# parsakhaz/multimodal-image-similarity-search

Hardware: AMD Instinct MI355X
Metric: images/s CLIP-B/32 encode @ bs256; Mvec/s cosine top-10 over 10M x 512 (higher is better)
Workload: dtype bf16

## Files before the change

### include/mmiss_debug.h

```cpp
#ifndef MMISS_DEBUG_H
#define MMISS_DEBUG_H
#include <stdint.h>
#ifdef __cplusplus
extern "C" {
#endif

enum {
    MMISS_EPI_F32 = 0,
    MMISS_EPI_BIAS_BF16 = 1,
    MMISS_EPI_BIAS_QGELU_BF16 = 2,
    MMISS_EPI_BIAS_RESID_F32 = 3,
    MMISS_EPI_PATCH_F32 = 4
};

int mmiss_dbg_gemm(int device, void* hip_stream, int epi, int variant, const void* A, const void* W,
                   void* out, const float* bias, const float* aux, int32_t M, int32_t N, int32_t K,
                   int32_t p0, int32_t p1);

int mmiss_dbg_layernorm(int device, void* hip_stream, const float* x, const float* gamma, const float* beta,
                        void* out, int32_t out_bf16, int32_t M, int32_t d, float eps);

int mmiss_dbg_attention(int device, void* hip_stream, const void* qkv, void* ctx, int32_t B, int32_t T,
                        int32_t H, int32_t causal);

int mmiss_dbg_attention_pooled(int device, void* hip_stream, const void* qkv, const int32_t* pool_row, void* ctxc, int32_t B,
                               int32_t T, int32_t H, int32_t causal);

int mmiss_dbg_gemm_resid_rows(int device, void* hip_stream, const void* A, const void* W, float* out, const float* bias,
                              const void* rows_bf16, const int32_t* rowmap, int32_t M, int32_t N, int32_t K);

int mmiss_dbg_patch_from_pixels(int device, void* hip_stream, const float* pixels, const void* W, float* out, const float* pos,
                                int32_t B, int32_t S, int32_t P, int32_t d);

int mmiss_dbg_im2col(int device, void* hip_stream, const float* pixels, void* out, int32_t B, int32_t S,
                     int32_t P, int32_t Kp);

int mmiss_dbg_gemm_time(int device, int epi, int variant, const void* A, const void* W, void* out,
                        const float* bias, const float* aux, int32_t M, int32_t N, int32_t K,
                        int32_t p0, int32_t p1, int32_t iters, float* ms_per_launch);

int mmiss_dbg_gemm_p256(int device, void* hip_stream, int epi, const void* A, const void* W, void* out,
                        const float* bias, const float* aux, const float* ln_stats, float ln_eps, int32_t M, int32_t N,
                        int32_t K, int32_t m_valid, int32_t iters, float* ms_per_launch);

int mmiss_dbg_gemm_resid16(int device, void* hip_stream, int variant, const void* A, const void* W, void* out,
                           const float* bias, float* stats_out, int32_t M, int32_t N, int32_t K, int32_t m_valid,
                           int32_t iters, float* ms_per_launch);

struct mmiss_encoder;
int mmiss_dbg_encoder_record_taps(struct mmiss_encoder* enc, int on);
int mmiss_dbg_encoder_set_fuse_ln(struct mmiss_encoder* enc, int on);

int mmiss_dbg_gemm_split_time(int device, int epi, int bm, const void* A, const void* W, void* out, const float* bias,
                              int32_t M, int32_t N, int32_t K, int32_t iters, float* ms);

int mmiss_dbg_quantize_weights_fp8(int device, void* hip_stream, const void* w_bf16, void* w8, float* scale, int32_t N,
                                   int32_t K);
int mmiss_dbg_layernorm_mxfp8(int device, void* hip_stream, const float* x, const float* gamma, const float* beta,
                              void* out8, void* out_scale, int32_t M, int32_t d, float eps);
int mmiss_dbg_layernorm16_mxfp8(int device, void* hip_stream, const void* x_bf16, const float* gamma, const float* beta,
                                void* out8, void* out_scale, int32_t M, int32_t d, float eps);
int mmiss_dbg_attention_mx(int device, void* hip_stream, const void* qkv, void* ctx8, void* ctx_scale, int32_t B, int32_t T,
                           int32_t H);
int mmiss_dbg_gemm8(int device, void* hip_stream, int epi, int bm, const void* A8, const void* As, const void* W8,
                    const float* wscale, const float* bias, void* out, void* out_scale, int32_t M, int32_t N, int32_t K);
int mmiss_dbg_gemm8_xt(int device, void* hip_stream, int epi, int xt, const void* A8, const void* As, const void* W8,
                       const float* wscale, const float* bias, void* out, void* out_scale, int32_t M, int32_t N, int32_t K,
                       int32_t m_valid, const void* c16, const float* ln_stats, const void* x16, float ln_eps, void* q_out,
                       void* q_scale, float* stats_out);
int mmiss_dbg_quant16_mxfp8_stats(int device, void* hip_stream, const void* x_bf16, void* out8, void* out_scale, float* stats,
                                  int32_t M, int32_t d);
int mmiss_dbg_quantize_weights_fp8_csum(int device, void* hip_stream, const void* w_bf16, void* w8, float* scale, void* c16,
                                        int32_t N, int32_t K);
int mmiss_dbg_gemm8_time(int device, int epi, int bm, const void* A8, const void* As, const void* W8, const float* wscale,
                         const float* bias, void* out, void* out_scale, int32_t M, int32_t N, int32_t K, int32_t iters,
                         float* ms_per_launch);

int mmiss_dbg_set_option(const char* key, int value);

#ifdef __cplusplus
}
#endif
#endif
```

### multimodal-image-similarity-search_amd/_lib.py

```python
from __future__ import annotations

import ctypes as C
import os
import threading

_HERE = os.path.dirname(os.path.abspath(__file__))
LIB_PATH = os.path.join(_HERE, "libmmiss.so")

MMISS_OK = 0
MMISS_F32 = 0
MMISS_F16 = 1
MMISS_F8 = 2
MMISS_PREC_BF16 = 0
MMISS_PREC_FP8 = 1
MMISS_PREC_BF16_F32RESID = 2
MMISS_TOWER_VISION = 0
MMISS_TOWER_TEXT = 1

EPI_F32, EPI_BIAS_BF16, EPI_BIAS_QGELU_BF16, EPI_BIAS_RESID_F32, EPI_PATCH_F32 = range(5)


class MmissError(RuntimeError):

    def __init__(self, code: int, msg: str):
# ... 27 lines not shown
    "mmiss_encoder_set_weight": (_I, [_P, C.c_char_p, _P, _I64, C.POINTER(_I)]),
    "mmiss_encoder_finalize": (_I, [_P]),
    "mmiss_encoder_set_precision": (_I, [_P, _I32]),
    "mmiss_encoder_set_tower_precision": (_I, [_P, _I32, _I32]),
    "mmiss_encoder_set_stream": (_I, [_P, _P, _I32]),
    "mmiss_encode_image": (_I, [_P, _P, _I32, _P]),
    "mmiss_encode_image_u8": (_I, [_P, _P, _I32, _P]),
    "mmiss_resize_crop_rgb": (_I, [_P, _P, _I64, _P, _P, _P, _I32, _P]),
    "mmiss_encode_image_rgb": (_I, [_P, _P, _I64, _P, _P, _P, _I32, _P]),
    "mmiss_encode_text": (_I, [_P, _P, _I32, _I32, _P]),
    "mmiss_encoder_tap": (_I, [_P, _I, _I, _P, _I64, C.POINTER(_I64)]),
    "mmiss_index_create": (_I, [_I32, _I32, _I, _I64, C.POINTER(_P)]),
    "mmiss_index_destroy": (_I, [_P]),
    "mmiss_index_set_stream": (_I, [_P, _P, _I32]),
    "mmiss_index_add": (_I, [_P, _P, _P, _I64]),
    "mmiss_index_update": (_I, [_P, _P, _P, _I64]),
    "mmiss_index_remove": (_I, [_P, _P, _I64, C.POINTER(_I64)]),
    "mmiss_index_clear": (_I, [_P]),
    "mmiss_index_count": (_I, [_P, C.POINTER(_I64)]),
    "mmiss_index_get": (_I, [_P, _P, _I64, _P]),
    "mmiss_index_labels": (_I, [_P, _P, _I64]),
    "mmiss_index_query": (_I, [_P, _P, _I32, _I32, _P, _P, _P]),
    "mmiss_index_query_begin": (_I, [_P, _P, _I32, _I32, _P, _P, _P]),
    "mmiss_index_query_end": (_I, [_P]),
    "mmiss_index_query_abort": (_I, [_P]),
    "mmiss_index_guard_stats": (_I, [_P, C.POINTER(_I64)]),
    "mmiss_index_guard_stats_ex": (_I, [_P, C.POINTER(_I64)]),
    "mmiss_index_save": (_I, [_P, C.c_char_p]),
    "mmiss_index_load": (_I, [_P, C.c_char_p]),
    "mmiss_index_set_tags": (_I, [_P, _P, _P, _I64]),
    "mmiss_index_get_tags": (_I, [_P, _P, _I64, _P]),
    "mmiss_index_query_filtered": (_I, [_P, _P, _I32, _I32, _P, _P, _P, _P, _P]),
    "mmiss_index_query_filtered_begin": (_I, [_P, _P, _I32, _I32, _P, _P, _P, _P, _P]),
    "mmiss_blend": (_I, [_I, _P, _P, _P, C.c_double, _I32, _I32, _P]),
    "mmiss_merge_topk": (_I, [_I, _P, _P, _P, _I32, _I32, _I32, _P, _P, _P]),
    "mmiss_prof_enable": (_I, [_I]),
    "mmiss_prof_filter": (_I, [C.c_char_p, _I]),
    "mmiss_prof_reset": (_I, []),
    "mmiss_prof_read": (_I, [C.c_char_p, C.c_size_t]),
    "mmiss_dbg_gemm": (_I, [_I, _P, _I, _I, _P, _P, _P, _P, _P, _I32, _I32, _I32, _I32, _I32]),
    "mmiss_dbg_gemm_p256": (_I, [_I, _P, _I, _P, _P, _P, _P, _P, _P, C.c_float, _I32, _I32, _I32, _I32, _I32, _P]),
    "mmiss_dbg_gemm_resid16": (_I, [_I, _P, _I, _P, _P, _P, _P, _P, _I32, _I32, _I32, _I32, _I32, _P]),
    "mmiss_dbg_gemm_time": (_I, [_I, _I, _I, _P, _P, _P, _P, _P, _I32, _I32, _I32, _I32, _I32, _I32,
                                 C.POINTER(C.c_float)]),
    "mmiss_dbg_layernorm": (_I, [_I, _P, _P, _P, _P, _P, _I32, _I32, _I32, C.c_float]),
    "mmiss_dbg_attention": (_I, [_I, _P, _P, _P, _I32, _I32, _I32, _I32]),
    "mmiss_dbg_im2col": (_I, [_I, _P, _P, _P, _I32, _I32, _I32, _I32]),
    "mmiss_dbg_patch_from_pixels": (_I, [_I, _P, _P, _P, _P, _P, _I32, _I32, _I32, _I32]),
    "mmiss_dbg_attention_pooled": (_I, [_I, _P, _P, _P, _P, _I32, _I32, _I32, _I32]),
    "mmiss_dbg_gemm_resid_rows": (_I, [_I, _P, _P, _P, _P, _P, _P, _P, _I32, _I32, _I32]),
    "mmiss_dbg_encoder_record_taps": (_I, [_P, _I]),
    "mmiss_dbg_encoder_set_fuse_ln": (_I, [_P, _I]),
    "mmiss_dbg_set_option": (_I, [C.c_char_p, _I]),
    "mmiss_dbg_quantize_weights_fp8": (_I, [_I, _P, _P, _P, _P, _I32, _I32]),
    "mmiss_dbg_layernorm_mxfp8": (_I, [_I, _P, _P, _P, _P, _P, _P, _I32, _I32, C.c_float]),
    "mmiss_dbg_layernorm16_mxfp8": (_I, [_I, _P, _P, _P, _P, _P, _P, _I32, _I32, C.c_float]),
    "mmiss_dbg_attention_mx": (_I, [_I, _P, _P, _P, _P, _I32, _I32, _I32]),
    "mmiss_dbg_gemm8": (_I, [_I, _P, _I, _I, _P, _P, _P, _P, _P, _P, _P, _I32, _I32, _I32]),
    "mmiss_dbg_gemm8_xt": (_I, [_I, _P, _I, _I, _P, _P, _P, _P, _P, _P, _P, _I32, _I32, _I32, _I32, _P, _P, _P, C.c_float, _P, _P, _P]),
    "mmiss_dbg_quant16_mxfp8_stats": (_I, [_I, _P, _P, _P, _P, _P, _I32, _I32]),
    "mmiss_dbg_quantize_weights_fp8_csum": (_I, [_I, _P, _P, _P, _P, _P, _I32, _I32]),
    "mmiss_dbg_gemm8_time": (_I, [_I, _I, _I, _P, _P, _P, _P, _P, _P, _P, _I32, _I32, _I32, _I32, C.POINTER(C.c_float)]),
    "mmiss_dbg_gemm_split_time": (_I, [_I, _I, _I, _P, _P, _P, _P, _I32, _I32, _I32, _I32, C.POINTER(C.c_float)]),
}

_lib = None
_lock = threading.Lock()


def load() -> C.CDLL:
    global _lib
    with _lock:
        if _lib is not None:
            return _lib
        if not os.path.exists(LIB_PATH):
            raise ImportError(
                f"{LIB_PATH} not found: the HIP extension is not built. "
                "Run `python -c 'import __graft_entry__ as g; g.build()'` at the repo root. "
                "There is no CPU fallback for the mmiss hot path."
            )
        lib = C.CDLL(LIB_PATH, mode=C.RTLD_GLOBAL)
        for name, (res, args) in SIGNATURES.items():
            fn = getattr(lib, name)
            fn.restype = res
            fn.argtypes = args
        if lib.mmiss_abi_version() != 1:
            raise ImportError("libmmiss.so ABI version mismatch")
        _lib = lib
        for kv in filter(None, os.environ.get("MMISS_OPTIONS", "").split(",")):
            k, _, v = kv.partition("=")
            lib.mmiss_dbg_set_option(k.strip().encode(), int(v))
        return lib


def check(status: int) -> None:
    if status != MMISS_OK:
        msg = load().mmiss_last_error()
        raise MmissError(status, msg.decode("utf-8", "replace") if msg else "")


def ptr(x) -> int:
    if x is None:
        return None
    if isinstance(x, int):
        return x
    if hasattr(x, "data_ptr"):
# ... 45 lines not shown
```

### multimodal-image-similarity-search_amd/csrc/api_index.hip

```cpp
#include "common.h"
#include <queue>
#include "retrieval_kernels.h"
#include "gemm_bf16_256.h"
#include "gemm_bf16_p256.h"
#include <algorithm>

struct mmiss_index {
    int dim = 0, dtype = MMISS_F32, device = 0, elt = 4;
    int qelt() const { return dtype == MMISS_F32 ? 4 : 2; }
    hipStream_t own_stream = nullptr, user_stream = nullptr;
    bool has_user_stream = false;
    hipEvent_t done_ev = nullptr;
    bool async_pending = false;
    std::mutex mu;
    int64_t count = 0, capacity = 0;
    DevBuf rows, labels_d;
    DevBuf inv;
    std::vector<int64_t> labels_h;
    DevBuf tags;
    std::vector<uint64_t> tags_h;
    DevBuf fmask, fmask2, tag_stage;
    DevBuf stage, qn, qs, qstage, lists_s, lists_r, lists2_s, lists2_r, cand, cur_s, cur_r, out_c, map, gmax;
    DevBuf qmap, qmap64, qs2, cand2;
    DevBuf eps_q, thr, thr2, swp_cnt, swp_list;
// ... 172 lines not shown
    int64_t target = std::max<int64_t>(1, (int64_t)256 * per_cu / p.qtiles);
    int64_t tpb = std::max<int64_t>(4, (((ntiles + target - 1) / target) + 3) / 4 * 4);
    p.tiles_per_block = (int)tpb;
    p.slabs = (int)((ntiles + tpb - 1) / tpb);
    return p;
}

typedef void (*ScanKernel)(ScanArgs);
template <typename T, bool THR, bool FILT>
ScanKernel scan_kernel(const ScanPlan& p) {
    if (p.nqt == 4) return &scan_topk_kernel<T, 4, 32, 8, THR, FILT>;
    if (p.nqt == 2) return &scan_topk_kernel<T, 2, 32, 8, THR, FILT>;
    if constexpr (std::is_same<T, _Float16>::value && !THR && !FILT)
        if (mmiss_option("scan_group", 8) == 16) return &scan_topk_kernel<T, 1, 64, 16, false, false>;
    return &scan_topk_kernel<T, 1, THR ? 32 : 64, 8, THR, FILT>;
}

int launch_scan(mmiss_index* ix, hipStream_t st, const ScanArgs& a, const ScanPlan& p) {
    const double flops = 2.0 * a.Q * (double)a.N * a.D;
    const double bytes = (p.thr ? (double)p.qtiles : 1.0) * a.N * a.D * ix->elt;
    const bool f16 = ix->dtype == MMISS_F16, f8 = ix->dtype == MMISS_F8;
    MM_PROF(p.thr ? (f16 ? "sweep_scan_f16" : f8 ? "sweep_scan_f8" : "sweep_scan_f32")
                  : (f16 ? "scan_topk_f16" : f8 ? "scan_topk_f8" : "scan_topk_f32"), st, flops, bytes);
    const ScanKernel kern = with_storage(ix->dtype, [&](auto s) {
        using T = typename decltype(s)::T;
        if (p.thr) return a.tags ? scan_kernel<T, true, true>(p) : scan_kernel<T, true, false>(p);
        return a.tags ? scan_kernel<T, false, true>(p) : scan_kernel<T, false, false>(p);
    });
    MM_TRY(mmiss_ensure_dyn_lds(reinterpret_cast<const void*>(kern), p.lds));
    hipLaunchKernelGGL(kern, dim3(p.slabs, p.qtiles), dim3(256), p.lds, st, a);
    MM_HIP(hipGetLastError());
    return MMISS_OK;
}

int launch_merge(mmiss_index* ix, hipStream_t st, MergeArgs m) {
    if (m.L > mmiss_option("merge_two_level_min", 64)) {
        const int per = 32;
        const int S = (m.L + per - 1) / per;
        MM_TRY(ix->lists2_s.ensure((size_t)S * m.Q * m.kp * 4));
        MM_TRY(ix->lists2_r.ensure((size_t)S * m.Q * m.kp * 4));
        MergeArgs m1 = m;
        m1.lists_per_block = per; m1.out_s = ix->lists2_s.as<float>(); m1.out_r = ix->lists2_r.as<int32_t>();
        m1.cur_s = nullptr; m1.cur_r = nullptr;
        {
            MM_PROF("merge_lists", st, 0.0, (double)m.L * m.Q * m.kp * 8);
            hipLaunchKernelGGL(merge_lists_kernel, dim3(m.Q, S), dim3(256), 0, st, m1);
            MM_HIP(hipGetLastError());
        }
        m.in_s = ix->lists2_s.as<float>(); m.in_r = ix->lists2_r.as<int32_t>(); m.L = S;
    }
    m.lists_per_block = 0; m.out_s = nullptr; m.out_r = nullptr;
    MM_PROF("merge_lists", st, 0.0, (double)m.L * m.Q * m.kp * 8);
    hipLaunchKernelGGL(merge_lists_kernel, dim3(m.Q), dim3(256), 0, st, m);
    MM_HIP(hipGetLastError());
    return MMISS_OK;
}

}

extern "C" int mmiss_index_create(int32_t dim, int32_t storage_dtype, int device, int64_t capacity_hint,
                                  mmiss_index** out) {
    if (!out) MM_FAIL(MMISS_ERR_ARG, "mmiss_index_create: null out");
    if (dim <= 0 || dim % 128 || dim > 4096) MM_FAIL(MMISS_ERR_UNSUPPORTED, "index dim %d: need a multiple of 128, <= 4096", dim);
    if (storage_dtype != MMISS_F32 && storage_dtype != MMISS_F16 && storage_dtype != MMISS_F8)
        MM_FAIL(MMISS_ERR_ARG, "unknown storage dtype %d", storage_dtype);
    if (scan_lds_bytes(dim, storage_dtype == MMISS_F32 ? 4 : 2, 1, 64) > SCAN_LDS_LIMIT)
        MM_FAIL(MMISS_ERR_UNSUPPORTED, "index dim %d with storage dtype %d: a 16-query block of the scan needs %d bytes of LDS (limit %d); "
                "f32 rows go up to dim 1920, f16 / fp8 rows up to 3968", dim, storage_dtype,
                scan_lds_bytes(dim, storage_dtype == MMISS_F32 ? 4 : 2, 1, 64), SCAN_LDS_LIMIT);
    MM_TRY(mmiss_use_device(device));
    mmiss_index* ix = new (std::nothrow) mmiss_index();
    if (!ix) MM_FAIL(MMISS_ERR_NOMEM, "out of host memory");
    ix->dim = dim; ix->dtype = storage_dtype; ix->device = device; ix->elt = storage_dtype == MMISS_F16 ? 2 : storage_dtype == MMISS_F8 ? 1 : 4;
    if (hipStreamCreateWithFlags(&ix->own_stream, hipStreamNonBlocking) != hipSuccess) {
        delete ix;
        MM_FAIL(MMISS_ERR_HIP, "hipStreamCreate failed");
    }
    if (hipEventCreateWithFlags(&ix->done_ev, hipEventDisableTiming) != hipSuccess) {
        (void)hipStreamDestroy(ix->own_stream);
        delete ix;
        MM_FAIL(MMISS_ERR_HIP, "hipEventCreate failed");
    }
    if (capacity_hint > 0) {
        int rc = index_reserve(ix, capacity_hint, ix->own_stream);
        if (rc != MMISS_OK) {
            (void)hipStreamDestroy(ix->own_stream); (void)hipEventDestroy(ix->done_ev);
            delete ix;
            return rc;
        }
    }
    *out = ix;
    return MMISS_OK;
}

extern "C" int mmiss_index_destroy(mmiss_index* ix) {
    if (!ix) return MMISS_OK;
    (void)hipSetDevice(ix->device);
    (void)hipDeviceSynchronize();
    if (ix->own_stream) (void)hipStreamDestroy(ix->own_stream);
    if (ix->done_ev) (void)hipEventDestroy(ix->done_ev);
    delete ix;
    return MMISS_OK;
}

extern "C" int mmiss_index_set_stream(mmiss_index* ix, void* hip_stream, int32_t use_own) {
    if (!ix) MM_FAIL(MMISS_ERR_ARG, "null index");
// ... 423 lines not shown
    const int SWEEP_FAST = 1024;
    RerankArgs r{};
    r.rows = ix->rows.p; r.D = D; r.inv = ix->inv.as<float>(); r.qn = ix->qn.as<float>(); r.cand = ix->swp_list.as<int32_t>();
    r.cand_stride = SWEEP_CAP; r.ncand = SWEEP_FAST; r.cand_cnt = ix->swp_cnt.as<int32_t>();
    r.group_mode = 0; r.nrows = N;
    r.labels = ix->labels_d.as<int64_t>(); r.k = pd.k;
    r.out_labels = pd.d_lab; r.out_dist = pd.d_dist; r.out_count = pd.d_cnt;
    r.qmap = qmap_sw;
    MM_TRY(ix->swp_pin.ensure((size_t)Qf * 4, st, (size_t)(Qf < 1024 ? 1024 : 2 * Qf) * 4));
    r.cnt_host = ix->swp_pin.as<int32_t>();
    MM_TRY(launch_rerank(ix, st, r, Qf));
    r.cnt_host = nullptr;
    MM_HIP(hipStreamSynchronize(st));
    const int32_t* cnt = ix->swp_pin.as<int32_t>();
    ix->stat_rounds += 1;
    std::vector<int32_t> big_b, rest;
    int maxc = 1;
    for (int b = 0; b < Qf; ++b) {
        if (cnt[b] > SWEEP_CAP) rest.push_back(which[b]);
        else {
            ix->stat_swept_rows += cnt[b];
            if (cnt[b] > SWEEP_FAST) { big_b.push_back(b); maxc = std::max(maxc, cnt[b]); }
        }
    }
    if (!big_b.empty()) {
        const int nb = (int)big_b.size();
        std::vector<int32_t> qm((size_t)nb);
        for (int j = 0; j < nb; ++j) qm[j] = which[big_b[j]];
        MM_TRY(ix->cand2.ensure((size_t)nb * 8));
        MM_HIP(hipMemcpyAsync(ix->cand2.p, big_b.data(), (size_t)nb * 4, hipMemcpyHostToDevice, st));
        MM_HIP(hipMemcpyAsync(ix->cand2.as<int32_t>() + nb, qm.data(), (size_t)nb * 4, hipMemcpyHostToDevice, st));
        MM_HIP(hipStreamSynchronize(st));
        r.ncand = (int)round_up(maxc, 32);
        r.bmap = ix->cand2.as<int32_t>();
        r.qmap = ix->cand2.as<int32_t>() + nb;
        MM_TRY(launch_rerank(ix, st, r, nb));
    }
    MM_TRY(exhaustive_queries(ix, st, pd, rest));
    MM_HIP(hipStreamSynchronize(st));
    return MMISS_OK;
}

}

namespace {

struct QueryPlan {
    int kp = 0, pages = 0, ncand = 0;
    bool dense = false;
    bool dense8 = false;
    bool big = false;
    bool strip_v3 = false;
    bool sample = false;
    int Mq = 0, strip = 1, filter_cap = 0;
    int64_t Npad = 0, nbn = 0, ns_tiles = 0, Ndense = 0;
};

int plan_query(const mmiss_index* ix, int Q, int k, bool filt, QueryPlan& p) {
    const int64_t N = ix->count;
    const int64_t want = std::min<int64_t>(k, N);
    if (want <= 10) { p.kp = 16; p.pages = 1; }
    else if (want <= 24) { p.kp = 32; p.pages = 1; }
    else {
        p.kp = 32;
        p.pages = (int)((std::min<int64_t>(want + 8, N) + 31) / 32);
    }
    p.ncand = p.kp * p.pages;
    if (p.ncand > 2048) MM_FAIL(MMISS_ERR_UNSUPPORTED, "mmiss_index_query: k = %d too large (max 2040)", k);

    const bool single = !filt && N > 0 && p.pages == 1;
    p.big = Q >= mmiss_option("score_big_min_q", 129);
    p.strip_v3 = strip_v3(ix);
    p.dense8 = single && ix->dtype == MMISS_F8 && p.big && p.strip_v3 && strip_gemm_rows(ix);
    p.dense = (single && ix->dtype == MMISS_F16 && Q > 16) || p.dense8;
    if (!p.dense) return MMISS_OK;
    p.Npad = round_up(N, p.big ? 256 : 128);
    p.Mq = (int)round_up(Q, p.big ? 256 : 128);
    p.nbn = p.Npad / 256;
    p.ns_tiles = std::max<int64_t>(16, p.nbn / std::max(1, mmiss_option("score_sample_div", 32)));
    const int filter_opt = mmiss_option("score_filter", 1);
    p.sample = p.big && p.nbn >= 128 && filter_opt != 0 && (filter_opt == 2 || (double)p.Mq * (double)p.Npad >= 1e9);
    p.Ndense = p.sample ? p.ns_tiles * 256 : p.Npad;
    if (p.big) p.strip = strip_length(p.Mq, p.nbn, p.sample ? p.nbn - p.ns_tiles : p.nbn);
    if (p.sample) p.filter_cap = mmiss_option("score_filter_cap", 2048);
    return MMISS_OK;
}

int stage_filter(mmiss_index* ix, hipStream_t st, int Q, const uint64_t* req, const uint64_t* exc) {
    mmiss_index::Pending& pd = ix->pend;
    pd.filt = req || exc;
    pd.d_mask = nullptr;
    if (!pd.filt) return MMISS_OK;
    if (req) MM_TRY(fetch_u64(req, Q, pd.req, st)); else pd.req.assign((size_t)Q, 0);
    if (exc) MM_TRY(fetch_u64(exc, Q, pd.exc, st)); else pd.exc.assign((size_t)Q, 0);
    MM_TRY(ix->fmask.ensure((size_t)Q * 16));
    MM_HIP(hipMemcpyAsync(ix->fmask.p, pd.req.data(), (size_t)Q * 8, hipMemcpyHostToDevice, st));
    MM_HIP(hipMemcpyAsync(ix->fmask.as<uint64_t>() + Q, pd.exc.data(), (size_t)Q * 8, hipMemcpyHostToDevice, st));
    pd.d_mask = ix->fmask.as<uint64_t>();
    return MMISS_OK;
}

int stage_outputs(mmiss_index* ix, hipStream_t st, int Q, int k, int64_t* out_labels, float* out_dist, int32_t* out_count) {
    mmiss_index::Pending& pd = ix->pend;
    pd.Q = Q; pd.k = k;
    const size_t pin_dist = (size_t)Q * k * 8, pin_cnt = pin_dist + (size_t)Q * k * 4, pin_flags = pin_cnt + (size_t)Q * 4;
    const size_t need = pin_flags + (size_t)Q * 4;
    size_t grow = 4096;
    while (grow < need) grow *= 2;
    MM_TRY(ix->pin.ensure(need, st, grow));
    char* const pin = ix->pin.as<char>();
    pd.d_lab = out_labels; pd.d_dist = out_dist; pd.d_cnt = out_count;
    if (!pd.out_dev) {
        pd.d_lab = reinterpret_cast<int64_t*>(pin); pd.d_dist = reinterpret_cast<float*>(pin + pin_dist);
        pd.d_cnt = reinterpret_cast<int32_t*>(pin + pin_cnt);
    } else if (!out_count) {
        MM_TRY(ix->out_c.ensure((size_t)Q * 4));
        pd.d_cnt = ix->out_c.as<int32_t>();
    }
    pd.h_flags = reinterpret_cast<int32_t*>(pin + pin_flags);
    pd.out_labels = out_labels; pd.out_dist = out_dist; pd.out_count = out_count;
    return MMISS_OK;
}

int upload_queries(mmiss_index* ix, hipStream_t st, const float* queries, int Q) {
    const int D = ix->dim;
    const int Qpad = (int)round_up(Q, 256);
    const float* qsrc = queries;
    if (!mmiss_is_device_ptr(queries)) {
        MM_TRY(ix->qstage.ensure((size_t)Q * D * 4));
        MM_HIP(hipMemcpyAsync(ix->qstage.p, queries, (size_t)Q * D * 4, hipMemcpyHostToDevice, st));
        qsrc = ix->qstage.as<float>();
    }
    MM_TRY(ix->qn.ensure((size_t)Qpad * D * 4));
    MM_TRY(ix->qs.ensure((size_t)Qpad * D * ix->qelt()));
    MM_TRY(ix->eps_q.ensure((size_t)Qpad * 4));
    MM_TRY(ix->thr.ensure((size_t)Qpad * 4));
    MM_PROF("prep_queries", st, 4.0 * Q * D, (double)Q * D * (8 + ix->elt));
    double eps_fixed, cnorm;
    guard_terms(ix, &eps_fixed, &cnorm);
    with_storage(ix->dtype, [&](auto s) {
        using QT = typename decltype(s)::Q;
        hipLaunchKernelGGL(prep_queries_kernel<QT>, dim3((Qpad + 3) / 4), dim3(256), 0, st, qsrc, ix->qn.as<float>(), ix->qs.as<QT>(),
                           Q, Qpad, D, ix->eps_q.as<float>(), eps_fixed, cnorm);
    });
    MM_HIP(hipGetLastError());
    return MMISS_OK;
}

int dense_pass(mmiss_index* ix, hipStream_t st, const QueryPlan& p, int Q) {
    const int D = ix->dim, kp = p.kp;
    const int64_t N = ix->count;
    const int ng = (int)(p.Ndense / 16);
    MM_TRY(ix->gmax.ensure((size_t)p.Mq * ng * 4));
    GemmEpi ep{};
    ep.out = ix->gmax.p; ep.ldo = ng; ep.m_valid = Q; ep.p0 = (int)N; ep.m_fast = 1;
    ep.aux = ix->inv.as<float>();
    {
        MM_PROF(p.dense8 ? (p.sample ? "score_gemm_f8_sample" : "score_gemm_f8") : (p.sample ? "score_gemm_f16_sample" : "score_gemm_f16"), st,
                2.0 * Q * (double)std::min<int64_t>(N, p.Ndense) * D, (double)std::min<int64_t>(N, p.Ndense) * D * ix->elt);
        if (p.big) MM_TRY(launch_strip_gemm(ix, st, p.strip_v3, ix->qs.p, ep, p.Mq, (int)p.Ndense, p.strip, nullptr));
        else MM_TRY((launch_gemm_inst<_Float16, 128, MMISS_EPI_GROUPMAX_F32>(st, ix->qs.p, ix->rows.p, ep, p.Mq, (int)p.Npad, D)));
    }
    const int units = (ng + 1023) / 1024;
    int splits = (1024 + Q - 1) / Q;
    if (splits > units) splits = units;
    if (splits > 32) splits = 32;
    if (splits < 1) splits = 1;
    MM_TRY(ix->lists_s.ensure((size_t)splits * Q * kp * 4));
    MM_TRY(ix->lists_r.ensure((size_t)splits * Q * kp * 4));
    SelectArgs sa{};
    sa.G = ix->gmax.as<float>(); sa.ldg = ng; sa.ng = ng; sa.kp = kp; sa.Q = Q;
    sa.out_s = ix->lists_s.as<float>(); sa.out_r = ix->lists_r.as<int32_t>();
    {
        MM_PROF("select_topk", st, 0.0, (double)Q * ng * 4);
        hipLaunchKernelGGL(select_topk_kernel, dim3(Q, splits), dim3(256), 0, st, sa);
        MM_HIP(hipGetLastError());
    }
    MergeArgs m{};
    m.in_s = ix->lists_s.as<float>(); m.in_r = ix->lists_r.as<int32_t>();
    m.L = splits; m.Q = Q; m.kp = kp;
    if (p.sample) {
        const int cap = p.filter_cap;
        MM_TRY(ix->seed_s.ensure((size_t)p.Mq * kp * 4));
        MM_TRY(ix->seed_r.ensure((size_t)p.Mq * kp * 4));
        MM_TRY(ix->fcnt.ensure((size_t)p.Mq * 4));
        MM_TRY(ix->fbuf_s.ensure((size_t)p.Mq * cap * 4));
        MM_TRY(ix->fbuf_g.ensure((size_t)p.Mq * cap * 4));
        {
            MergeArgs m1 = m;
            m1.lists_per_block = splits; m1.out_s = ix->seed_s.as<float>(); m1.out_r = ix->seed_r.as<int32_t>();
            MM_PROF("merge_lists", st, 0.0, (double)splits * Q * kp * 8);
            hipLaunchKernelGGL(merge_lists_kernel, dim3(Q, 1), dim3(256), 0, st, m1);
            MM_HIP(hipGetLastError());
        }
        MM_HIP(hipMemsetAsync(ix->fcnt.p, 0, (size_t)p.Mq * 4, st));
        StripFilter flt{};
        flt.tau = ix->seed_s.as<float>() + (kp - 1); flt.tau_stride = kp;
        flt.cnt = ix->fcnt.as<int32_t>(); flt.buf_s = ix->fbuf_s.as<float>(); flt.buf_g = ix->fbuf_g.as<int32_t>();
        flt.cap = cap; flt.bn_begin = (int)p.ns_tiles;
        {
            MM_PROF(p.dense8 ? "score_gemm_f8" : "score_gemm_f16", st, 2.0 * Q * (double)(N - p.Ndense) * D, (double)(N - p.Ndense) * D * ix->elt);
            MM_TRY(launch_strip_gemm(ix, st, p.strip_v3, ix->qs.p, ep, p.Mq, (int)p.Npad, p.strip, &flt));
        }
        m.in_s = ix->seed_s.as<float>(); m.in_r = ix->seed_r.as<int32_t>(); m.L = 1;
        m.flat_s = ix->fbuf_s.as<float>(); m.flat_r = ix->fbuf_g.as<int32_t>(); m.flat_cnt = ix->fcnt.as<int32_t>();
        m.flat_cap = cap;
    }
    m.cand = ix->cand.as<int32_t>(); m.cand_stride = p.ncand; m.page_off = 0;
    m.cur_s = ix->cur_s.as<float>(); m.cur_r = ix->cur_r.as<int32_t>();
    return launch_merge(ix, st, m);
}

int scan_pass(mmiss_index* ix, hipStream_t st, const QueryPlan& qp, int Q) {
    const mmiss_index::Pending& pd = ix->pend;
// ... 119 lines not shown
extern "C" int mmiss_index_query(mmiss_index* ix, const float* queries, int32_t Q, int32_t k, int64_t* out_labels,
                                 float* out_dist, int32_t* out_count) {
    return query_entry(ix, queries, Q, k, nullptr, nullptr, out_labels, out_dist, out_count, false, "mmiss_index_query");
}

extern "C" int mmiss_index_query_begin(mmiss_index* ix, const float* queries, int32_t Q, int32_t k, int64_t* out_labels,
                                       float* out_dist, int32_t* out_count) {
    return query_entry(ix, queries, Q, k, nullptr, nullptr, out_labels, out_dist, out_count, true, "mmiss_index_query_begin");
}

extern "C" int mmiss_index_query_filtered(mmiss_index* ix, const float* queries, int32_t Q, int32_t k, const uint64_t* require,
                                          const uint64_t* exclude, int64_t* out_labels, float* out_dist, int32_t* out_count) {
    return query_entry(ix, queries, Q, k, require, exclude, out_labels, out_dist, out_count, false, "mmiss_index_query_filtered");
}

extern "C" int mmiss_index_query_filtered_begin(mmiss_index* ix, const float* queries, int32_t Q, int32_t k, const uint64_t* require,
                                                const uint64_t* exclude, int64_t* out_labels, float* out_dist, int32_t* out_count) {
    return query_entry(ix, queries, Q, k, require, exclude, out_labels, out_dist, out_count, true, "mmiss_index_query_filtered_begin");
}

extern "C" int mmiss_index_query_end(mmiss_index* ix) {
    if (!ix) MM_FAIL(MMISS_ERR_ARG, "mmiss_index_query_end: null index");
    std::lock_guard<std::mutex> lk(ix->mu);
    if (!ix->pend.active) MM_FAIL(MMISS_ERR_STATE, "mmiss_index_query_end: no query was begun");
    return query_end_locked(ix);
}

extern "C" int mmiss_index_query_abort(mmiss_index* ix) {
    if (!ix) MM_FAIL(MMISS_ERR_ARG, "mmiss_index_query_abort: null index");
    std::lock_guard<std::mutex> lk(ix->mu);
    if (!ix->pend.active) return MMISS_OK;
    ix->pend.active = false;
    MM_TRY(mmiss_use_device(ix->device));
    MM_HIP(hipEventSynchronize(ix->done_ev));
    return MMISS_OK;
}

extern "C" int mmiss_index_guard_stats_ex(mmiss_index* ix, int64_t out[8]) {
    if (!ix || !out) MM_FAIL(MMISS_ERR_ARG, "mmiss_index_guard_stats_ex: null argument");
    std::lock_guard<std::mutex> lk(ix->mu);
    for (int i = 0; i < 8; ++i) out[i] = 0;
    out[0] = ix->stat_queries; out[1] = ix->stat_flagged; out[2] = ix->stat_rounds; out[3] = ix->stat_pages;
    out[4] = ix->stat_exhaustive; out[5] = ix->stat_swept_rows;
    return MMISS_OK;
}

extern "C" int mmiss_index_guard_stats(mmiss_index* ix, int64_t out[4]) {
    if (!ix || !out) MM_FAIL(MMISS_ERR_ARG, "mmiss_index_guard_stats: null argument");
    std::lock_guard<std::mutex> lk(ix->mu);
    out[0] = ix->stat_queries; out[1] = ix->stat_flagged; out[2] = ix->stat_rounds; out[3] = ix->stat_pages;
    return MMISS_OK;
}

namespace {
struct IdxHeader {
    char magic[8];
    int32_t version, dim, dtype, reserved;
    int64_t count;
};

int load_rows(mmiss_index* ix, FILE* f, const char* path, int64_t n, const std::vector<int64_t>& lab, hipStream_t st) {
    const size_t row_bytes = (size_t)ix->dim * ix->elt;
    const int64_t chunk = std::max<int64_t>(1, (64 << 20) / (int64_t)row_bytes);
    std::vector<char> buf((size_t)std::min<int64_t>(chunk, std::max<int64_t>(n, 1)) * row_bytes);
    for (int64_t r0 = 0; r0 < n; r0 += chunk) {
        const int64_t nr = std::min(chunk, n - r0);
        if (fread(buf.data(), row_bytes, (size_t)nr, f) != (size_t)nr ||
            hipMemcpy(ix->rows.as<char>() + (size_t)r0 * row_bytes, buf.data(), (size_t)nr * row_bytes, hipMemcpyHostToDevice) != hipSuccess)
            MM_FAIL(MMISS_ERR_IO, "%s could not be read to its end", path);
    }
    if (n) MM_HIP(hipMemcpy(ix->labels_d.p, lab.data(), (size_t)n * 8, hipMemcpyHostToDevice));
    if (ix->dtype == MMISS_F8 && ix->capacity > 0) {
        MM_HIP(hipMemsetAsync(ix->inv.p, 0, (size_t)ix->capacity * 4, st));
        MM_TRY(launch_f8_inv(ix, 0, n, st));
        MM_HIP(hipStreamSynchronize(st));
    }
    if (ix->capacity > 0) {
        MM_HIP(hipMemsetAsync(ix->tags.p, 0, (size_t)ix->capacity * 8, st));
        MM_HIP(hipStreamSynchronize(st));
    }
    return MMISS_OK;
}
}

extern "C" int mmiss_index_save(mmiss_index* ix, const char* path) {
    if (!ix || !path) MM_FAIL(MMISS_ERR_ARG, "mmiss_index_save: null argument");
    std::lock_guard<std::mutex> lk(ix->mu);
    MM_NO_PENDING(ix, "mmiss_index_save");
    MM_TRY(mmiss_use_device(ix->device));
    MM_HIP(hipStreamSynchronize(ix->stream()));
    FILE* f = fopen(path, "wb");
    if (!f) MM_FAIL(MMISS_ERR_IO, "cannot open %s for writing", path);
    IdxHeader h{};
    memcpy(h.magic, "MMISSIDX", 8);
    h.version = 1; h.dim = ix->dim; h.dtype = ix->dtype; h.count = ix->count;
    bool ok = fwrite(&h, sizeof(h), 1, f) == 1;
    if (ok && ix->count) ok = fwrite(ix->labels_h.data(), 8, (size_t)ix->count, f) == (size_t)ix->count;
    const size_t row_bytes = (size_t)ix->dim * ix->elt;
    const int64_t chunk = std::max<int64_t>(1, (64 << 20) / (int64_t)row_bytes);
    std::vector<char> buf((size_t)std::min<int64_t>(chunk, std::max<int64_t>(ix->count, 1)) * row_bytes);
    for (int64_t r0 = 0; ok && r0 < ix->count; r0 += chunk) {
        const int64_t nr = std::min(chunk, ix->count - r0);
        if (hipMemcpy(buf.data(), ix->rows.as<char>() + (size_t)r0 * row_bytes, (size_t)nr * row_bytes,
                      hipMemcpyDeviceToHost) != hipSuccess) { ok = false; break; }
        ok = fwrite(buf.data(), row_bytes, (size_t)nr, f) == (size_t)nr;
    }
// ... 135 lines not shown
```

### multimodal-image-similarity-search_amd/csrc/retrieval_kernels.h

```cpp
#pragma once
#include "common.h"
#include "gemm_bf16.h"
#include <math.h>
#include <type_traits>

#define SCAN_NEG_INF (-INFINITY)
#define SCAN_ROW_NONE 0x7fffffff

__device__ __forceinline__ double wave_butterfly_sum(double v) {
#pragma unroll
    for (int o = 32; o > 0; o >>= 1) v = v + __shfl_xor(v, o);
    return v;
}

#define MMISS_F8_SCALE 128.0f
struct F8 {
    uint8_t b;
    F8() = default;
    __device__ explicit F8(float y) { b = (uint8_t)(__builtin_amdgcn_cvt_pk_fp8_f32(y * MMISS_F8_SCALE, 0.0f, 0, false) & 0xff); }
    __device__ explicit operator float() const { return __builtin_amdgcn_cvt_f32_fp8((int)b, 0) * (1.0f / MMISS_F8_SCALE); }
};
__device__ __forceinline__ void f8x4_values(uint32_t w, float (&v)[4]) {
    v[0] = __builtin_amdgcn_cvt_f32_fp8((int)w, 0) * (1.0f / MMISS_F8_SCALE);
    v[1] = __builtin_amdgcn_cvt_f32_fp8((int)w, 1) * (1.0f / MMISS_F8_SCALE);
// ... 609 lines not shown
            cs[wave][pos] = s;
            cr[wave][pos] = r;
        }
        __builtin_amdgcn_fence(__ATOMIC_SEQ_CST, "wavefront");
        const int c = cnt[wave];
        if (c > kp) {
            float ss = SCAN_NEG_INF;
            int rr = SCAN_ROW_NONE;
            if (lane < c) { ss = cs[wave][lane]; rr = cr[wave][lane]; }
            wave_sort64(ss, rr, lane);
            if (lane < kp) { cs[wave][lane] = ss; cr[wave][lane] = rr; }
            tau = __shfl(ss, kp - 1);
            if (lane == 0) cnt[wave] = kp;
            __builtin_amdgcn_fence(__ATOMIC_SEQ_CST, "wavefront");
        }
        e0 = e1;
        s = sn;
        r = rn;
    }
    __syncthreads();
    if (wave == 0) {
        float s = SCAN_NEG_INF;
        int r = SCAN_ROW_NONE;
        const int c0 = cnt[0];
        if (lane < c0) { s = cs[0][lane]; r = cr[0][lane]; }
        wave_sort64(s, r, lane);
        for (int w = 1; w < 4; ++w) {
            const int cw = cnt[w];
            if (cw == 0) continue;
            if (lane >= kp) { s = SCAN_NEG_INF; r = SCAN_ROW_NONE; }
            if (lane >= 32 && lane - 32 < cw) { s = cs[w][lane - 32]; r = cr[w][lane - 32]; }
            wave_sort64(s, r, lane);
        }
        const bool valid = lane < kp && r != SCAN_ROW_NONE;
        if (a.out_s) {
            if (lane < kp) {
                const size_t o = ((size_t)blockIdx.y * a.Q + q) * kp + lane;
                a.out_s[o] = valid ? s : SCAN_NEG_INF;
                a.out_r[o] = valid ? r : -1;
            }
            return;
        }
        if (lane < kp) a.cand[(size_t)q * a.cand_stride + a.page_off + lane] = valid ? r : -1;
        if (a.cur_s) {
            const unsigned long long m = __ballot(valid);
            const int nvalid = __popcll(m);
            const float ls = __shfl(s, nvalid > 0 ? nvalid - 1 : 0);
            const int lr = __shfl(r, nvalid > 0 ? nvalid - 1 : 0);
            if (lane == 0) {
                if (nvalid == kp) { a.cur_s[q] = ls; a.cur_r[q] = lr; }
                else { a.cur_s[q] = SCAN_NEG_INF; a.cur_r[q] = SCAN_ROW_NONE; }
            }
        }
    }
}

struct RerankArgs {
    const void* rows; int D;
    const float* qn;
    const int32_t* cand;
    int cand_stride, ncand;
    int group_mode;
    int64_t nrows;
    const int64_t* labels;
    int k;
    int64_t* out_labels;
    float* out_dist;
    int32_t* out_count;
    const int32_t* qmap;
    int32_t* out_rows;
    const float* tau;
    double eps;
    int32_t* flags;
    int32_t* nflag;
    int force_flag;
    const int32_t* ovf_cnt;
    int ovf_cap;
    const float* eps_q;
    float* thr_out;
    const int32_t* cand_cnt;
    const int32_t* bmap;
    const float* inv;
    int32_t* cnt_host;
};

template <typename T>
__device__ __forceinline__ void canon_partial_dots(const T* rv, bool live, const float* qp, int D, double (&acc)[4]) {
    acc[0] = acc[1] = acc[2] = acc[3] = 0.0;
    typedef typename std::conditional<sizeof(T) == 1, uint32_t, typename std::conditional<sizeof(T) == 2, u32x2, f32x4>::type>::type piece_t;
    for (int d0 = 0; d0 < D; d0 += 512) {
        piece_t w[8];
        f32x4 qq[8];
#pragma unroll
        for (int u = 0; u < 8; ++u) {
            w[u] = piece_t{};
            qq[u] = f32x4{0.f, 0.f, 0.f, 0.f};
            if (d0 + 64 * u < D) {
                qq[u] = *reinterpret_cast<const f32x4*>(qp + d0 + 64 * u);
                if (live) w[u] = *reinterpret_cast<const piece_t*>(rv + d0 + 64 * u);
            }
        }
#pragma unroll
        for (int u = 0; u < 8; ++u) {
            if (d0 + 64 * u < D) {
                float rr[4];
                if constexpr (sizeof(T) == 1) {
// ... 287 lines not shown
```

Baseline: 89550.

## Fuse group top-k selection into single-pass threshold-filter kernel per query

Measured after the change: 90390 (median of 3 runs). No clear change (+0.9%).

```diff
diff --git a/include/mmiss_debug.h b/include/mmiss_debug.h
--- a/include/mmiss_debug.h
+++ b/include/mmiss_debug.h
@@ -76,6 +76,9 @@
                          const float* bias, void* out, void* out_scale, int32_t M, int32_t N, int32_t K, int32_t iters,
                          float* ms_per_launch);
 
+int mmiss_dbg_select_groups(int device, void* hip_stream, const float* G, int32_t ldg, int32_t ng, int32_t Q, int32_t kp,
+                            int32_t* cand, float* cur_s, int32_t* cur_r);
+
 int mmiss_dbg_set_option(const char* key, int value);
 
 #ifdef __cplusplus
diff --git a/multimodal-image-similarity-search_amd/_lib.py b/multimodal-image-similarity-search_amd/_lib.py
--- a/multimodal-image-similarity-search_amd/_lib.py
+++ b/multimodal-image-similarity-search_amd/_lib.py
@@ -103,6 +103,7 @@
     "mmiss_dbg_encoder_record_taps": (_I, [_P, _I]),
     "mmiss_dbg_encoder_set_fuse_ln": (_I, [_P, _I]),
     "mmiss_dbg_set_option": (_I, [C.c_char_p, _I]),
+    "mmiss_dbg_select_groups": (_I, [_I, _P, _P, _I32, _I32, _I32, _I32, _P, _P, _P]),
     "mmiss_dbg_quantize_weights_fp8": (_I, [_I, _P, _P, _P, _P, _I32, _I32]),
     "mmiss_dbg_layernorm_mxfp8": (_I, [_I, _P, _P, _P, _P, _P, _P, _I32, _I32, C.c_float]),
     "mmiss_dbg_layernorm16_mxfp8": (_I, [_I, _P, _P, _P, _P, _P, _P, _I32, _I32, C.c_float]),
diff --git a/multimodal-image-similarity-search_amd/csrc/api_index.hip b/multimodal-image-similarity-search_amd/csrc/api_index.hip
--- a/multimodal-image-similarity-search_amd/csrc/api_index.hip
+++ b/multimodal-image-similarity-search_amd/csrc/api_index.hip
@@ -248,6 +248,16 @@
     m.lists_per_block = 0; m.out_s = nullptr; m.out_r = nullptr;
     MM_PROF("merge_lists", st, 0.0, (double)m.L * m.Q * m.kp * 8);
     hipLaunchKernelGGL(merge_lists_kernel, dim3(m.Q), dim3(256), 0, st, m);
+    MM_HIP(hipGetLastError());
+    return MMISS_OK;
+}
+
+int launch_select_groups(hipStream_t st, const SelectGroupsArgs& a, int Q) {
+    if (a.kp < 1 || a.kp > 32 || a.ng < 1 || a.ldg < a.ng || a.ldg % 4 || a.cand_stride < a.kp || (reinterpret_cast<uintptr_t>(a.G) & 15))
+        MM_FAIL(MMISS_ERR_ARG, "select_groups: ng=%d ldg=%d kp=%d stride=%d", a.ng, a.ldg, a.kp, a.cand_stride);
+    MM_PROF("select_groups", st, 0.0, (double)Q * a.ng * 4);
+    if (a.ng <= SELG_CHUNK) hipLaunchKernelGGL(select_groups_kernel<true>, dim3(Q), dim3(SELG_THREADS), 0, st, a);
+    else hipLaunchKernelGGL(select_groups_kernel<false>, dim3(Q), dim3(SELG_THREADS), 0, st, a);
     MM_HIP(hipGetLastError());
     return MMISS_OK;
 }
@@ -777,6 +787,7 @@
     bool big = false;
     bool strip_v3 = false;
     bool sample = false;
+    bool fused = false;
     int Mq = 0, strip = 1, filter_cap = 0;
     int64_t Npad = 0, nbn = 0, ns_tiles = 0, Ndense = 0;
 };
@@ -808,6 +819,7 @@
     p.Ndense = p.sample ? p.ns_tiles * 256 : p.Npad;
     if (p.big) p.strip = strip_length(p.Mq, p.nbn, p.sample ? p.nbn - p.ns_tiles : p.nbn);
     if (p.sample) p.filter_cap = mmiss_option("score_filter_cap", 2048);
+    p.fused = !p.sample && mmiss_option("select_fused", 1) != 0 && p.Npad / 16 <= mmiss_option("select_fused_max_ng", 65536);
     return MMISS_OK;
 }
 
@@ -885,6 +897,13 @@
                 2.0 * Q * (double)std::min<int64_t>(N, p.Ndense) * D, (double)std::min<int64_t>(N, p.Ndense) * D * ix->elt);
         if (p.big) MM_TRY(launch_strip_gemm(ix, st, p.strip_v3, ix->qs.p, ep, p.Mq, (int)p.Ndense, p.strip, nullptr));
         else MM_TRY((launch_gemm_inst<_Float16, 128, MMISS_EPI_GROUPMAX_F32>(st, ix->qs.p, ix->rows.p, ep, p.Mq, (int)p.Npad, D)));
+    }
+    if (p.fused) {
+        SelectGroupsArgs sg{};
+        sg.G = ix->gmax.as<float>(); sg.ldg = ng; sg.ng = ng; sg.kp = kp;
+        sg.cand = ix->cand.as<int32_t>(); sg.cand_stride = p.ncand;
+        sg.cur_s = ix->cur_s.as<float>(); sg.cur_r = ix->cur_r.as<int32_t>();
+        return launch_select_groups(st, sg, Q);
     }
     const int units = (ng + 1023) / 1024;
     int splits = (1024 + Q - 1) / Q;
@@ -1110,6 +1129,40 @@
     return MMISS_OK;
 }
 
+extern "C" int mmiss_dbg_select_groups(int device, void* hip_stream, const float* G, int32_t ldg, int32_t ng, int32_t Q, int32_t kp,
+                                       int32_t* cand, float* cur_s, int32_t* cur_r) {
+    if (!G || !cand || !cur_s || !cur_r) MM_FAIL(MMISS_ERR_ARG, "mmiss_dbg_select_groups: null pointer");
+    if (Q < 1 || ng < 1 || ldg < ng || ldg % 4 || (kp != 16 && kp != 32)) MM_FAIL(MMISS_ERR_ARG, "mmiss_dbg_select_groups: Q=%d ng=%d ldg=%d kp=%d", Q, ng, ldg, kp);
+    MM_TRY(mmiss_use_device(device));
+    hipStream_t st = reinterpret_cast<hipStream_t>(hip_stream);
+    if (mmiss_option("select_fused", 1) != 0) {
+        SelectGroupsArgs sg{};
+        sg.G = G; sg.ldg = ldg; sg.ng = ng; sg.kp = kp; sg.cand = cand; sg.cand_stride = kp; sg.cur_s = cur_s; sg.cur_r = cur_r;
+        return launch_select_groups(st, sg, Q);
+    }
+    int splits = std::max(1, std::min(std::min((1024 + Q - 1) / Q, (ng + 1023) / 1024), 32));
+    void* lists = nullptr;
+    const size_t half = (size_t)splits * Q * kp * 4;
+    MM_HIP(hipMallocAsync(&lists, 2 * half, st));
+    SelectArgs sa{};
+    sa.G = G; sa.ldg = ldg; sa.ng = ng; sa.kp = kp; sa.Q = Q;
+    sa.out_s = static_cast<float*>(lists); sa.out_r = reinterpret_cast<int32_t*>(static_cast<char*>(lists) + half);
+    {
+        MM_PROF("select_topk", st, 0.0, (double)Q * ng * 4);
+        hipLaunchKernelGGL(select_topk_kernel, dim3(Q, splits), dim3(256), 0, st, sa);
+    }
+    MergeArgs m{};
+    m.in_s = sa.out_s; m.in_r = sa.out_r; m.L = splits; m.Q = Q; m.kp = kp;
+    m.cand = cand; m.cand_stride = kp; m.cur_s = cur_s; m.cur_r = cur_r;
+    {
+        MM_PROF("merge_lists", st, 0.0, (double)splits * Q * kp * 8);
+        hipLaunchKernelGGL(merge_lists_kernel, dim3(Q), dim3(256), 0, st, m);
+    }
+    MM_HIP(hipGetLastError());
+    MM_HIP(hipFreeAsync(lists, st));
+    return MMISS_OK;
+}
+
 namespace {
 struct IdxHeader {
     char magic[8];
diff --git a/multimodal-image-similarity-search_amd/csrc/retrieval_kernels.h b/multimodal-image-similarity-search_amd/csrc/retrieval_kernels.h
--- a/multimodal-image-similarity-search_amd/csrc/retrieval_kernels.h
+++ b/multimodal-image-similarity-search_amd/csrc/retrieval_kernels.h
@@ -685,6 +685,166 @@
                 else { a.cur_s[q] = SCAN_NEG_INF; a.cur_r[q] = SCAN_ROW_NONE; }
             }
         }
+    }
+}
+
+#define SELG_THREADS 512
+#define SELG_CHUNK (SELG_THREADS * 16)
+#define SELG_CAP 1024
+
+struct SelectGroupsArgs {
+    const float* G;
+    int ldg;
+    int ng;
+    int kp;
+    int32_t* cand;
+    int cand_stride;
+    float* cur_s;
+    int32_t* cur_r;
+};
+
+__device__ __forceinline__ uint32_t selg_score_bits(float s) {
+    const uint32_t u = __float_as_uint(s);
+    return u ^ ((u >> 31) ? 0xffffffffu : 0x80000000u);
+}
+__device__ __forceinline__ uint64_t selg_key(float s, int id) {
+    return s > SCAN_NEG_INF ? ((uint64_t)selg_score_bits(s) << 32) | (uint32_t)~id : 0ull;
+}
+
+__device__ __forceinline__ void selg_load(const float* __restrict__ row, int ng, int c0, int tid, f32x4 (&v)[4]) {
+#pragma unroll
+    for (int j = 0; j < 4; ++j) {
+        const int c = c0 + j * (SELG_THREADS * 4) + tid * 4;
+        f32x4 x = {SCAN_NEG_INF, SCAN_NEG_INF, SCAN_NEG_INF, SCAN_NEG_INF};
+        if (c + 3 < ng) {
+            x = *reinterpret_cast<const f32x4*>(row + c);
+        } else {
+#pragma unroll
+            for (int e = 0; e < 4; ++e)
+                if (c + e < ng) x[e] = row[c + e];
+        }
+        v[j] = x;
+    }
+}
+__device__ __forceinline__ void selg_clean(f32x4 (&v)[4]) {
+#pragma unroll
+    for (int j = 0; j < 4; ++j)
+#pragma unroll
+        for (int e = 0; e < 4; ++e) v[j][e] = v[j][e] > SCAN_NEG_INF ? v[j][e] + 0.0f : SCAN_NEG_INF;
+}
+
+template <bool SINGLE>
+__global__ __launch_bounds__(SELG_THREADS) void select_groups_kernel(SelectGroupsArgs a) {
+    __shared__ __attribute__((aligned(16))) uint64_t lk[SELG_CAP];
+    __shared__ float wb[SELG_THREADS / 64];
+    __shared__ int cnts[3];
+    __shared__ int nsurv;
+    const int tid = threadIdx.x, lane = tid & 63, wave = tid >> 6;
+    const int q = blockIdx.x, kp = a.kp, ng = a.ng;
+    const float* row = a.G + (size_t)q * a.ldg;
+    if (tid == 0) { nsurv = 0; cnts[0] = 0; cnts[1] = 0; cnts[2] = 0; }
+
+    f32x4 v0[4];
+    if constexpr (SINGLE) { selg_load(row, ng, 0, tid, v0); selg_clean(v0); }
+    auto each = [&](auto&& fn) {
+        if constexpr (SINGLE) {
+            fn(v0, 0);
+        } else {
+            f32x4 v[4], vn[4];
+            selg_load(row, ng, 0, tid, v);
+            for (int c0 = 0; c0 < ng; c0 += SELG_CHUNK) {
+                if (c0 + SELG_CHUNK < ng) selg_load(row, ng, c0 + SELG_CHUNK, tid, vn);
+                selg_clean(v);
+                fn(v, c0);
+#pragma unroll
+                for (int j = 0; j < 4; ++j) v[j] = vn[j];
+            }
+        }
+    };
+    auto file = [&](const f32x4 (&v)[4], int c0, float B, uint64_t T) {
+#pragma unroll
+        for (int j = 0; j < 4; ++j)
+#pragma unroll
+            for (int e = 0; e < 4; ++e) {
+                const float s = v[j][e];
+                const uint64_t key = selg_key(s, c0 + j * (SELG_THREADS * 4) + tid * 4 + e);
+                const bool take = key != 0 && s >= B && key >= T;
+                const unsigned long long mk = __ballot(take);
+                if (mk) {
+                    const int first = __ffsll((long long)mk) - 1;
+                    int base = 0;
+                    if (lane == first) base = atomicAdd(&nsurv, __popcll(mk));
+                    base = __shfl(base, first);
+                    const int pos = base + __popcll(mk & ((1ull << lane) - 1ull));
+                    if (take && pos < SELG_CAP) lk[pos] = key;
+                }
+            }
+    };
+
+    float m = SCAN_NEG_INF;
+    each([&](const f32x4 (&v)[4], int) {
+#pragma unroll
+        for (int j = 0; j < 4; ++j) m = fmaxf(m, fmaxf(fmaxf(v[j][0], v[j][1]), fmaxf(v[j][2], v[j][3])));
+    });
+    {
+        int r = lane;
+        wave_sort64(m, r, lane);
+        const float kth = __shfl(m, kp - 1);
+        if (lane == 0) wb[wave] = kth;
+    }
+    __syncthreads();
+    float B = wb[0];
+#pragma unroll
+    for (int w = 1; w < SELG_THREADS / 64; ++w) B = fmaxf(B, wb[w]);
+
+    each([&](const f32x4 (&v)[4], int c0) { file(v, c0, B, 0ull); });
+    __syncthreads();
+    int S = nsurv;
+    if (S > SELG_CAP) {
+        uint64_t T = 0;
+        for (int it = 0; it < 64; ++it) {
+            const uint64_t t = T | (1ull << (63 - it));
+            int c = 0;
+            each([&](const f32x4 (&v)[4], int c0) {
+#pragma unroll
+                for (int j = 0; j < 4; ++j)
+#pragma unroll
+                    for (int e = 0; e < 4; ++e) c += selg_key(v[j][e], c0 + j * (SELG_THREADS * 4) + tid * 4 + e) >= t;
+            });
+#pragma unroll
+            for (int o = 32; o > 0; o >>= 1) c += __shfl_xor(c, o);
+            if (lane == 0 && c) atomicAdd(&cnts[it % 3], c);
+            if (tid == 0) cnts[(it + 1) % 3] = 0;
+            __syncthreads();
+            if (cnts[it % 3] >= kp) T = t;
+        }
+        if (tid == 0) nsurv = 0;
+        __syncthreads();
+        each([&](const f32x4 (&v)[4], int c0) { file(v, c0, SCAN_NEG_INF, T); });
+        __syncthreads();
+        S = nsurv;
+    }
+    if (tid == 0 && (S & 1)) lk[S] = 0ull;
+    __syncthreads();
+
+    int32_t* cand = a.cand + (size_t)q * a.cand_stride;
+    for (int t = tid; t < S; t += SELG_THREADS) {
+        const uint64_t mine = lk[t];
+        int rank = 0;
+#pragma unroll 4
+        for (int j = 0; j < S; j += 2) {
+            const ulonglong2 kk = *reinterpret_cast<const ulonglong2*>(&lk[j]);
+            rank += (kk.x > mine) + (kk.y > mine);
+        }
+        if (rank < kp) {
+            const int id = (int)~(uint32_t)mine;
+            cand[rank] = id;
+            if (rank == kp - 1) { a.cur_s[q] = row[id]; a.cur_r[q] = id; }
+        }
+    }
+    if (S < kp) {
+        if (tid >= S && tid < kp) cand[tid] = -1;
+        if (tid == 0) { a.cur_s[q] = SCAN_NEG_INF; a.cur_r[q] = SCAN_ROW_NONE; }
     }
 }
 
```
